# zicodasilva/cheetah_pose_estimation

Measured on AMD Instinct MI355X. Metric: frames/sec residual+Jacobian eval + full-traj solves/sec, 200-frame 6-cam seq, higher is better.
Workload: dtype f64; 1 GPU; cfg2: synthetic 200-frame x 6-cam x 25-marker sequences, phantom skeleton, const-accel model; frames=200, cams=6, markers=25, sequences_per_gpu=2048, parallelism=shard1 (independent sequences, no collective)

## Files before the change

cheetah_pose_estimation_amd/csrc/cpe_api.hip:

```cpp
#include <hip/hip_runtime.h>

#include <cmath>
#include <cstdio>
#include <cstdlib>
#include <cstring>
#include <functional>
#include <string>
#include <vector>
#include <algorithm>
#include <type_traits>

#include "cpe_kernels.hip"

static thread_local std::string g_err;
static cpe_status fail(cpe_status s, const std::string& m) { g_err = m; return s; }
#define HIPCHK(x)                                                                                         \
    do {                                                                                                  \
        hipError_t e_ = (x);                                                                              \
        if (e_ != hipSuccess) return fail(CPE_HIP_ERROR, std::string(#x) + ": " + hipGetErrorString(e_)); \
    } while (0)

struct cpe_handle {
    int device = 0;
    int n_cu = 256;
// ... 407 lines not shown
    return CPE_OK;
}

static void build_com_model(const cpe_skeleton* s, const cpe_camera* cams, int C, const cpe_options* o, std::vector<DevModel>& out, std::string& err) {
    if (!err.empty()) return;
    cpe_skeleton c = *s;
    c.n_markers = s->n_links;
    for (int i = 0; i < s->n_links && i < CPE_MAX_MARKERS; i++) {
        c.marker_link[i] = i;
        for (int d = 0; d < 3; d++) c.marker_off[i][d] = s->com[i][d];
    }
    const std::string keep = g_err;
    out.emplace_back();
    if (build_model(&c, cams, C, o, out.back(), false) != CPE_OK) { err = g_err; out.clear(); }
    g_err = keep;
}

template <bool RAGGED = false>
static auto frame_normal(bool plain) { return plain ? k_frame_normal<true, RAGGED> : k_frame_normal<false, RAGGED>; }
static size_t lds_fk(const DevModel& m) { return sizeof(double) * (m.nq + 6 * m.nl + 36 * m.nl + 3 * m.L + 23 * m.C); }
static size_t lds_normal(const DevModel& m, int gmm_k = 0, int gmm_dim = 0, bool shutter = false) {
    const bool plain = gmm_k == 0 && !shutter;
    size_t ov = CPE_MAX_SCOL * m.n_srow, hg = plain ? m.nu : m.nu * m.nu + m.nu;
    size_t camov = 6 * m.nl + 2 * m.nrev + 36 * m.n_trunk;
    if (camov < (size_t)22 * m.C) camov = (size_t)22 * m.C;
    size_t n = m.ns + camov + 3 * m.L + 3 * m.sv_n + GAM_STRIDE * m.nrev + (ov > hg ? ov : hg) +
               9 * m.L + 3 * m.mc_total;
    if (gmm_k > 0) n += CPE_NX + gmm_k * gmm_dim + CPE_MAX_GMM + CPE_NX;
    if (shutter) n += 15 * m.C + 6 * m.L + 6;
    return sizeof(double) * n;
}
template <bool RAGGED = false>
static auto frame_tracked(bool gmm) { return gmm ? k_frame_tracked<true, RAGGED> : k_frame_tracked<false, RAGGED>; }
static size_t lds_tracked(const DevModel& m, int gmm_k, int gmm_dim) {
    size_t n = m.ns + 6 * m.nl + 2 * m.nrev + 36 * m.n_trunk + GAM_STRIDE * m.nrev + m.nu + m.nu * m.nu + m.nu;
    if (gmm_k > 0) n += CPE_NX + gmm_k * gmm_dim + CPE_MAX_GMM + CPE_NX;
    return sizeof(double) * n;
}
template <class Fn>
static size_t lds_all(const cpe_handle* h, Fn&& lds) {
    size_t n = lds(h->hm);
    for (const DevModel& m : h->models) n = std::max(n, lds(m));
    return n;
}
static size_t lds_normal_all(const cpe_handle* h) { return lds_all(h, [h](const DevModel& m) { return lds_normal(m, h->gmm_k, h->gmm_dim); }); }
static size_t lds_fk(const cpe_handle* h, const RaggedArgs* rg) { return rg ? lds_all(h, [](const DevModel& m) { return lds_fk(m); }) : lds_fk(h->hm); }
static size_t lds_normal(const cpe_handle* h, const RaggedArgs* rg, bool shutter = false) {
    return rg ? lds_normal_all(h) : lds_normal(h->hm, h->gmm_k, h->gmm_dim, shutter);
}
static size_t lds_tracked(const cpe_handle* h, const RaggedArgs* rg) {
    return rg ? lds_all(h, [h](const DevModel& m) { return lds_tracked(m, h->gmm_k, h->gmm_dim); }) : lds_tracked(h->hm, h->gmm_k, h->gmm_dim);
}
static int n_models(const cpe_handle* h) { return h->models.empty() ? 1 : (int)h->models.size(); }
static int cams_max(const cpe_handle* h) {
    int c = h->hm.C;
    for (const DevModel& m : h->models) c = std::max(c, m.C);
    return c;
}

extern "C" {

const char* cpe_last_error(void) { return g_err.c_str(); }

void cpe_default_options(cpe_options* o) {
    o->h = 1.0 / 120.0; o->loss_a = 3.0; o->loss_b = 10.0; o->loss_c = 20.0; o->cost_scale = 1e-3;
    o->bound_penalty = 1e4; o->bound_tol = 1e-6; o->lambda0 = 1e-4; o->tol_step = 1e-8; o->tol_cost = 1e-9; o->max_iter = 200;
    o->curvature = 0; o->max_outer = 8; o->_pad = 0;
}

void cpe_destroy(cpe_handle* h);
static cpe_status create_impl(cpe_handle* h, const cpe_skeleton* skel, const cpe_camera* cams, int32_t n_cams, const cpe_options* opts,
                              const cpe_priors* priors, bool use_pri, const std::vector<DevModel>* models = nullptr) {
    const int device = h->device;
    if (models) { h->models = *models; h->hm = h->models[0]; }
    else {
        if (cpe_status s = build_model(skel, cams, n_cams, opts, h->hm); s != CPE_OK) return s;
        build_com_model(skel, cams, n_cams, opts, h->cmodels, h->com_err);
    }
    HIPCHK(hipSetDevice(device));
    {
        hipDeviceProp_t prop;
        HIPCHK(hipGetDeviceProperties(&prop, device));
        h->n_cu = prop.multiProcessorCount > 0 ? prop.multiProcessorCount : 256;
        const void* ks[] = {(const void*)&k_resjac<true, 4, 3, 2>, (const void*)&k_resjac<false, 4, 3, 2>,
                            (const void*)&k_resjac<true, 4, 4, 2>, (const void*)&k_resjac<false, 4, 4, 2>,
                            (const void*)&k_dyn_eval<>, (const void*)&k_dyn_assemble<>, (const void*)&k_dyn_schur<>, (const void*)&k_dyn_jac<>,
                            (const void*)&k_dyn_eval<true>, (const void*)&k_dyn_assemble<true>, (const void*)&k_dyn_schur<true>, (const void*)&k_dyn_jac<true>,
                            (const void*)&k_force_cov<>, (const void*)&k_force_cov<true>};
        for (const void* k : ks) {
            hipFuncAttributes fa;
            HIPCHK(hipFuncGetAttributes(&fa, k));
            HIPCHK(hipFuncSetAttribute(k, hipFuncAttributeMaxDynamicSharedMemorySize, 160 * 1024 - (int)fa.sharedSizeBytes));
        }
    }
    HIPCHK(hipStreamCreateWithFlags(&h->stream, hipStreamNonBlocking));
    HIPCHK(hipEventCreateWithFlags(&h->order_ev, hipEventDisableTiming));
    for (int i = 0; i < 2; i++) HIPCHK(hipEventCreateWithFlags(&h->poll_ev[i], hipEventDisableTiming));
    HIPCHK(hipHostMalloc(reinterpret_cast<void**>(&h->poll_host), 2 * sizeof(int), hipHostMallocDefault));
    HIPCHK(hipMalloc(&h->n_act, sizeof(int)));
    HIPCHK(hipMalloc(&h->dm, sizeof(DevModel) * n_models(h)));
    HIPCHK(hipMemcpy(h->dm, h->models.empty() ? &h->hm : h->models.data(), sizeof(DevModel) * n_models(h), hipMemcpyHostToDevice));
    HIPCHK(hipMalloc(&h->flag, sizeof(int)));
    if (!h->cmodels.empty()) {
        HIPCHK(hipMalloc(&h->dmc, sizeof(DevModel) * h->cmodels.size()));
        HIPCHK(hipMemcpy(h->dmc, h->cmodels.data(), sizeof(DevModel) * h->cmodels.size(), hipMemcpyHostToDevice));
    }
    if (use_pri) {
        if (h->hm.nu != CPE_NX) return fail(CPE_BAD_ARG, "learned priors need the 28 relative angles of the reference's skeleton");
        if (priors->gmm_k > 0 && priors->gmm_dim > h->hm.nu) return fail(CPE_BAD_ARG, "pose prior dimension exceeds the number of relative angles");
        std::vector<DevPriors> hp(1);
        DevPriors& P = hp[0];
        memset(&P, 0, sizeof(P));
        P.p = *priors;
        const int W = priors->lr_window, nu = CPE_NX;
        if (W > 0) {
            auto K = [&](int t, int p2, int j) -> double { return t == W ? (p2 == j ? 1.0 : 0.0) : -priors->lr_coef[p2][t * nu + j]; };
            for (int ta = 0; ta <= W; ta++)
                for (int tb = 0; tb <= ta; tb++)
                    for (int i = 0; i < nu; i++)
                        for (int j = 0; j < nu; j++) {
                            double a = 0.0;
                            for (int p2 = 0; p2 < nu; p2++) a += K(ta, p2, i) * priors->lr_w[p2] * K(tb, p2, j);
                            P.lr_PK[ta][tb][i * nu + j] = 2.0 * a;
                        }
            for (int k = 0; k <= W; k++)
                for (int ta = k; ta <= W; ta++)
                    for (int e = 0; e < nu * nu; e++) P.lr_HI[k][e] += P.lr_PK[ta][ta - k][e];
            for (int f = 0; f < W * nu; f++) {
                bool any = false;
                for (int p2 = 0; p2 < nu; p2++) { P.lr_coefT[f][p2] = priors->lr_coef[p2][f]; any = any || priors->lr_coef[p2][f] != 0.0; }
                if (any) P.lr_feat[P.lr_nf++] = (uint8_t)f;
            }
        }
        const DevModel& hm = h->hm;
        for (int i = 0; i < nu; i++)
            for (int side = 0; side < 2; side++) {
                const int kk = side == 0 ? i : hm.rel_ref_u[i];
                if (kk < 0) continue;
                const double sgn = side == 0 ? hm.rel_sign_u[i] : -hm.rel_sign_u[i];
                P.Xc[i][kk] += sgn;
                const int r = hm.rev_of_u[kk];
                if (r >= 0) P.Xc[i][hm.rev_body_u[r][1]] += sgn;
            }
        auto to_u = [&](const double* A, double* out) {
            std::vector<double> T((size_t)nu * nu);
            for (int r2 = 0; r2 < nu; r2++)
                for (int j = 0; j < nu; j++) { double a = 0.0; for (int c = 0; c < nu; c++) a += A[r2 * nu + c] * P.Xc[c][j]; T[(size_t)r2 * nu + j] = a; }
            for (int i = 0; i < nu; i++)
                for (int j = 0; j < nu; j++) { double a = 0.0; for (int r2 = 0; r2 < nu; r2++) a += P.Xc[r2][i] * T[(size_t)r2 * nu + j]; out[i * nu + j] = a; }
        };
        if (W > 0) {
            for (int ta = 0; ta <= W; ta++) for (int tb = 0; tb <= ta; tb++) to_u(P.lr_PK[ta][tb], P.lr_PKu[ta][tb]);
            for (int k = 0; k <= W; k++) to_u(P.lr_HI[k], P.lr_HIu[k]);
        }
        if (priors->gmm_k > 0) {
            const int D = priors->gmm_dim, off = nu - D;
            std::vector<double> A((size_t)nu * nu);
            for (int k = 0; k < priors->gmm_k; k++) {
                std::fill(A.begin(), A.end(), 0.0);
                for (int i = 0; i < D; i++)
                    for (int j = 0; j < D; j++) { A[(size_t)(off + i) * nu + off + j] = priors->gmm_P[k][i][j]; P.gmm_PT[k][j][i] = priors->gmm_P[k][i][j]; }
                to_u(A.data(), P.gmm_Q[k]);
            }
        }
        HIPCHK(hipMalloc(&h->pri, sizeof(DevPriors)));
        HIPCHK(hipMemcpy(h->pri, &P, sizeof(DevPriors), hipMemcpyHostToDevice));
        h->gmm_k = priors->gmm_k; h->gmm_dim = priors->gmm_dim; h->lr_window = W;
        h->pb = W > 3 ? W : 3;
// ... 122 lines not shown
cpe_status cpe_synchronize(cpe_handle* h) {
    if (!h) return fail(CPE_BAD_ARG, "null handle");
    HIPCHK(hipStreamSynchronize(h->stream));
    return CPE_OK;
}

cpe_status cpe_stream_wait(cpe_handle* h, void* other) {
    if (!h) return fail(CPE_BAD_ARG, "null handle");
    HIPCHK(hipSetDevice(h->device));
    HIPCHK(hipEventRecord(h->order_ev, (hipStream_t)other));
    HIPCHK(hipStreamWaitEvent(h->stream, h->order_ev, 0));
    return CPE_OK;
}
cpe_status cpe_stream_signal(cpe_handle* h, void* other) {
    if (!h) return fail(CPE_BAD_ARG, "null handle");
    HIPCHK(hipSetDevice(h->device));
    HIPCHK(hipEventRecord(h->order_ev, h->stream));
    HIPCHK(hipStreamWaitEvent((hipStream_t)other, h->order_ev, 0));
    return CPE_OK;
}

cpe_status cpe_profile_enable(cpe_handle* h, int32_t on) {
    if (!h) return fail(CPE_BAD_ARG, "null handle");
    h->prof = on != 0;
    for (int i = 0; i < CPE_PROFILE_SLOTS; i++) { h->prof_ms[i] = 0.0; h->prof_n[i] = 0; }
    return CPE_OK;
}
cpe_status cpe_profile_get(cpe_handle* h, double* ms, int64_t* launches) {
    if (!h || !ms || !launches) return fail(CPE_BAD_ARG, "null argument");
    for (int i = 0; i < CPE_PROFILE_SLOTS; i++) { ms[i] = h->prof_ms[i]; launches[i] = h->prof_n[i]; }
    return CPE_OK;
}
static void prof_begin(cpe_handle* h, int id) {
    if (!h->prof) return;
    hipEvent_t a = nullptr, b = nullptr;
    if (hipEventCreate(&a) != hipSuccess || hipEventCreate(&b) != hipSuccess) return;
    (void)hipEventRecord(a, h->stream);
    h->prof_spans.push_back({id, {a, b}});
}
static void prof_end(cpe_handle* h) {
    if (!h->prof || h->prof_spans.empty()) return;
    (void)hipEventRecord(h->prof_spans.back().second.second, h->stream);
}
static void prof_collect(cpe_handle* h) {
    for (auto& sp : h->prof_spans) {
        float ms = 0.f;
        if (hipEventElapsedTime(&ms, sp.second.first, sp.second.second) == hipSuccess) { h->prof_ms[sp.first] += ms; h->prof_n[sp.first]++; }
        (void)hipEventDestroy(sp.second.first); (void)hipEventDestroy(sp.second.second);
    }
    h->prof_spans.clear();
}

int32_t cpe_jacobian_slots(const cpe_handle* h) { return h ? h->hm.S : 0; }
cpe_status cpe_jacobian_layout(const cpe_handle* h, int32_t* slot_marker, int32_t* slot_dof) {
    if (!h || !slot_marker || !slot_dof) return fail(CPE_BAD_ARG, "null argument");
    for (int s = 0; s < h->hm.S; s++) { slot_marker[s] = h->hm.slot_marker[s]; slot_dof[s] = h->hm.slot_dof[s]; }
    return CPE_OK;
}
int32_t cpe_num_independent(const cpe_handle* h) { return h ? h->hm.nu : 0; }
cpe_status cpe_independent_dofs(const cpe_handle* h, int32_t* dofs) {
    if (!h || !dofs) return fail(CPE_BAD_ARG, "null argument");
    for (int k = 0; k < h->hm.nu; k++) dofs[k] = h->hm.indep[k];
    return CPE_OK;
}

static cpe_status frames(int32_t B, int32_t N, size_t* F) {
    if (B < 0 || N < 0) return fail(CPE_BAD_ARG, "negative size");
    *F = (size_t)B * N;
    if (*F > 0x7fffffffULL) return fail(CPE_BAD_ARG, "too many frames for one launch");
    return CPE_OK;
}

cpe_status cpe_eval_resjac(cpe_handle* h, int32_t B, int32_t N, const double* q, const double* meas, const double* weight,
                           double* r, double* J, double* eps, double* cost) {
    if (!h || !q || !meas || !r || !J || !eps) return fail(CPE_BAD_ARG, "null argument");
    if (cost && !weight) return fail(CPE_BAD_ARG, "cost requested without weights");
    size_t F;
    if (cpe_status s = frames(B, N, &F); s != CPE_OK) return s;
    if (F == 0) return CPE_OK;
    HIPCHK(hipSetDevice(h->device));
    const DevModel& m = h->hm;
    if (m.C * m.L > RJ_MAXPASS * WAVE) return fail(CPE_BAD_ARG, "cpe_eval_resjac supports at most 256 (camera, marker) pairs");
    constexpr int NW = 4;
    const size_t lds = sizeof(double) * (((rj_shared_doubles(m.C, m.L, m.S) + 1) & ~1) + (size_t)NW * rj_wave_doubles(m.C, m.L, m.nq, m.nl));
    int wg_per_cu = (int)((160 * 1024) / lds);
    if (wg_per_cu < 1) return fail(CPE_BAD_ARG, "model too large for the LDS of one workgroup");
    constexpr int variant = 2;
    if (wg_per_cu > variant) wg_per_cu = variant;
    long grid = (long)h->n_cu * wg_per_cu;
    const long need = (long)((F + NW - 1) / NW);
    if (grid > need) grid = need;
    const int npass = (m.C * m.L + WAVE - 1) / WAVE;
#define RJ_LAUNCH(COST, NP, OC) hipLaunchKernelGGL((k_resjac<COST, NW, NP, OC>), dim3((unsigned)grid), dim3(WAVE * NW), lds, h->stream, h->dm, N, (long)F, q, meas, weight, r, J, eps, cost)
    if (cost) { if (npass <= 3) RJ_LAUNCH(true, 3, 2); else RJ_LAUNCH(true, 4, 2); }
    else { if (npass <= 3) RJ_LAUNCH(false, 3, 2); else RJ_LAUNCH(false, 4, 2); }
#undef RJ_LAUNCH
    HIPCHK(hipGetLastError());
    return CPE_OK;
}

cpe_status cpe_project_joints(cpe_handle* h, int32_t B, int32_t N, double* q) {
    if (!h || !q) return fail(CPE_BAD_ARG, "null argument");
    size_t F;
    if (cpe_status s = frames(B, N, &F); s != CPE_OK) return s;
    if (F == 0) return CPE_OK;
    HIPCHK(hipSetDevice(h->device));
    HIPCHK(hipMemsetAsync(h->flag, 0, sizeof(int), h->stream));
    hipLaunchKernelGGL(k_project, dim3((unsigned)F), dim3(WAVE), sizeof(double) * (h->hm.nq + 6 * h->hm.nl), h->stream, h->dm, q, h->flag);
    HIPCHK(hipGetLastError());
    int fl = 0;
    HIPCHK(hipMemcpyAsync(&fl, h->flag, sizeof(int), hipMemcpyDeviceToHost, h->stream));
    HIPCHK(hipStreamSynchronize(h->stream));
    return fl ? CPE_NUMERICAL : CPE_OK;
}

cpe_status cpe_grf_fit(cpe_handle* h, const cpe_grf_options* opt, int32_t B, int32_t N, const double* q, const double* dq,
                       const double* ddq, const int32_t* contact, double* grfz, double* grfxy, double* residual) {
    if (!h || !opt || !q || !dq || !ddq || !contact || !grfz || !grfxy) return fail(CPE_BAD_ARG, "null argument");
    size_t F;
    if (cpe_status s = frames(B, N, &F); s != CPE_OK) return s;
    if (opt->n_feet < 1 || opt->n_feet > 4 || opt->iterations < 1 || !(opt->gravity > 0) || !(opt->force_max > 0) || !(opt->friction_ratio >= 0))
        return fail(CPE_BAD_ARG, "grf options out of range");
    for (int f = 0; f < opt->n_feet; f++)
        if (opt->foot_marker[f] < 0 || opt->foot_marker[f] >= h->hm.L) return fail(CPE_BAD_ARG, "foot marker index out of range");
    if (F == 0) return CPE_OK;
    HIPCHK(hipSetDevice(h->device));
    hipLaunchKernelGGL(k_grf, dim3((unsigned)((F + GRF_PACK - 1) / GRF_PACK)), dim3(WAVE), 0, h->stream, h->dm, *opt, F, q, dq, ddq, contact, grfz, grfxy, residual);
    HIPCHK(hipGetLastError());
    return CPE_OK;
}

cpe_status cpe_eom_rows(cpe_handle* h, const cpe_eom_options* opt, int32_t B, int32_t N, const double* q, const double* dq,
                        const double* ddq, double* rows) {
    if (!h || !opt || !q || !dq || !ddq || !rows) return fail(CPE_BAD_ARG, "null argument");
    size_t F;
    if (cpe_status s = frames(B, N, &F); s != CPE_OK) return s;
    if (F == 0) return CPE_OK;
    HIPCHK(hipSetDevice(h->device));
    if (!h->eom) HIPCHK(hipMalloc(&h->eom, sizeof(cpe_eom_options)));
    HIPCHK(hipMemcpyAsync(h->eom, opt, sizeof(cpe_eom_options), hipMemcpyHostToDevice, h->stream));
    hipLaunchKernelGGL(k_eom, dim3((unsigned)F), dim3(WAVE), 0, h->stream, h->dm, h->eom, F, q, dq, ddq, rows);
    HIPCHK(hipGetLastError());
    return CPE_OK;
}

cpe_status cpe_eom_residual(cpe_handle* h, const cpe_dyn_options* opt, int32_t B, int32_t N, const double* q, const double* dq,
                            const double* ddq, const double* tau, const double* lambda, const double* grf, double* residual) {
    if (!h || !opt || !q || !dq || !ddq || !residual) return fail(CPE_BAD_ARG, "null argument");
    if (opt->n_feet < 0 || opt->n_feet > 4 || opt->n_motors < 0 || opt->n_motors > 32) return fail(CPE_BAD_ARG, "dynamics options out of range");
    for (int f = 0; f < opt->n_feet; f++) if (opt->foot_marker[f] < 0 || opt->foot_marker[f] >= h->hm.L) return fail(CPE_BAD_ARG, "foot marker index out of range");
    for (int m = 0; m < opt->n_motors; m++)
        if (opt->motor_first[m] < 0 || opt->motor_first[m] >= h->hm.nl || opt->motor_second[m] < 0 || opt->motor_second[m] >= h->hm.nl ||
            opt->motor_axis[m] < 0 || opt->motor_axis[m] > 2) return fail(CPE_BAD_ARG, "motor definition out of range");
    size_t F;
    if (cpe_status s = frames(B, N, &F); s != CPE_OK) return s;
    cpe_status s = cpe_eom_rows(h, &opt->eom, B, N, q, dq, ddq, residual);
    if (s != CPE_OK) return s;
    if (F == 0 || (!tau && !lambda && !grf)) return CPE_OK;
    if (!h->dyn) HIPCHK(hipMalloc(&h->dyn, sizeof(cpe_dyn_options)));
    HIPCHK(hipMemcpyAsync(h->dyn, opt, sizeof(cpe_dyn_options), hipMemcpyHostToDevice, h->stream));
    int n_con = 0;
    for (int j = 0; j < h->hm.nj; j++) n_con += h->hm.joint_kind[j] == CPE_JOINT_REVOLUTE_Y ? 2 : 1;
    hipLaunchKernelGGL(k_dyn_forces, dim3((unsigned)F), dim3(WAVE), 0, h->stream, h->dm, h->dyn, F, q, tau, lambda, grf, n_con, residual);
    HIPCHK(hipGetLastError());
    return CPE_OK;
}

cpe_status cpe_forward_kinematics(cpe_handle* h, int32_t B, int32_t N, const double* q, double* positions, double* com) {
    if (!h || !q || !positions) return fail(CPE_BAD_ARG, "null argument");
    size_t F;
    if (cpe_status s = frames(B, N, &F); s != CPE_OK) return s;
    if (F == 0) return CPE_OK;
    HIPCHK(hipSetDevice(h->device));
    hipLaunchKernelGGL(k_fk, dim3((unsigned)F), dim3(WAVE), lds_fk(h->hm), h->stream, h->dm, q, positions, com);
    HIPCHK(hipGetLastError());
    return CPE_OK;
}

cpe_status cpe_marker_velocities(cpe_handle* h, int32_t B, int32_t N, const double* q, const double* dq, double* velocities) {
// ... 1784 lines not shown
```

cheetah_pose_estimation_amd/csrc/cpe_kernels.hip:

```cpp
#include <hip/hip_runtime.h>

#include "cpe_device.h"


__device__ __forceinline__ void wave_sincos(const DevModel* __restrict__ M, const double* sq, double* ssc, int lane) {
    if (lane < 3 * M->nl) {
        double s, c;
        sincos(sq[3 + lane], &s, &c);
        ssc[2 * lane] = s; ssc[2 * lane + 1] = c;
    }
}

__device__ __forceinline__ void wave_rotations(const DevModel* __restrict__ M, const double* ssc, double* sR, int lane) {
    for (int t = lane; t < 4 * M->nl; t += WAVE) rot_kind(ssc + 6 * (t >> 2), t & 3, sR + 9 * t);
}

__device__ __forceinline__ void wave_markers(const DevModel* __restrict__ M, const double* sq, const double* sR,
                                             double* spos, int lane) {
    if (lane < M->L) {
        double p0 = sq[0], p1 = sq[1], p2 = sq[2];
        const int n = M->chain_len[lane];
        for (int k = 0; k < n; k++) {
            const double* R = sR + 36 * M->chain_link[lane][k];
            const double v0 = M->chain_vec[lane][k][0], v1 = M->chain_vec[lane][k][1], v2 = M->chain_vec[lane][k][2];
// ... 74 lines not shown
__device__ __forceinline__ void wave_tail_roll(double* sq, double* ssc, int hj_n, int fwx, int lane) {
    for (int level = 0; level < 2; level++) {
        if (lane < hj_n && ((fwx >> 16) & 1) == level) {
            const int p = fwx & 255, c = (fwx >> 8) & 255;
            double a[3], phi, sphi, cphi;
            rot_ycol(ssc + 6 * p, a);
            hooke_roll(a, ssc[6 * c + 2], ssc[6 * c + 3], ssc[6 * c + 4], ssc[6 * c + 5], phi, sphi, cphi);
            sq[3 + 3 * c] = phi;
            ssc[6 * c] = sphi; ssc[6 * c + 1] = cphi;
        }
        wave_lds_sync();
    }
}

__device__ __forceinline__ void wave_trunk_rotations(const DevModel* __restrict__ M, const double* ssc, double* sR, int fwy, int lane) {
    if (lane < 4 * M->n_trunk) rot_kind(ssc + 6 * fwy, lane & 3, sR + 9 * lane);
    for (int t = WAVE + lane; t < 4 * M->n_trunk; t += WAVE) rot_kind(ssc + 6 * M->trunk_link[t >> 2], t & 3, sR + 9 * t);
}

__device__ __forceinline__ void wave_leg_vectors(const double* ssa, double* sdyn, int svn, int fww, const double (&svv)[3][3], int lane) {
    if (lane < svn) {
        double d0 = 0.0, d1 = 0.0, d2 = 0.0;
        if ((fww & 3) == 0) {
            const int cnt = (fww >> 2) & 3;
#pragma unroll
            for (int i = 0; i < 3; i++) {
                const int r = (fww >> (4 + 6 * i)) & 63;
                const double sa = ssa[2 * r], ca = ssa[2 * r + 1];
                if (i < cnt) { d0 += ca * svv[i][0] + sa * svv[i][2]; d1 += svv[i][1]; d2 += -sa * svv[i][0] + ca * svv[i][2]; }
            }
        } else {
            const int r = (fww >> 4) & 63;
            const double sa = ssa[2 * r], ca = ssa[2 * r + 1];
            d0 = -sa * svv[0][0] + ca * svv[0][2]; d2 = -ca * svv[0][0] - sa * svv[0][2];
        }
        sdyn[3 * lane] = d0; sdyn[3 * lane + 1] = d1; sdyn[3 * lane + 2] = d2;
    }
}

__device__ __forceinline__ void wave_hooke_srows(const double* sR, double* sSv, int hk_n, int2 hkw, int lane) {
    for (int level = 0; level < 2; level++) {
        if (lane < hk_n && ((hkw.x >> 16) & 1) == level) {
            const double* Rp = sR + 36 * (hkw.x & 63); const double* Rc = sR + 36 * ((hkw.x >> 6) & 63);
            const double y0 = Rp[1], y1 = Rp[4], y2 = Rp[7];
            const double z0 = Rc[2], z1 = Rc[5], z2 = Rc[8];
            const double* Dcphi = Rc + 9;
            const double gphi = y0 * Dcphi[2] + y1 * Dcphi[5] + y2 * Dcphi[8];
            const int kind = (hkw.x >> 12) & 3, ang = (hkw.x >> 14) & 3;
            double direct = 0.0;
            if (kind == 0) { const double* D = Rc + 9 * (1 + ang); direct = y0 * D[2] + y1 * D[5] + y2 * D[8]; }
            else if (kind == 1) { const double* D = Rp + 9 * (1 + ang); direct = D[1] * z0 + D[4] * z1 + D[7] * z2; }
            double val = -direct / gphi;
            const int ch = (hkw.y & 0xFFFF) - 1;
            if (ch >= 0) {
                const double* Dpphi = Rp + 9;
                const double t0 = -(Dpphi[1] * z0 + Dpphi[4] * z1 + Dpphi[7] * z2) / gphi;
                val += t0 * sSv[ch];
            }
            sSv[hkw.y >> 16] = val;
        }
        wave_lds_sync();
    }
}

#define RJ_MAXPASS 4

#define RJ_GLOBAL __attribute__((address_space(1)))
typedef double rj_v2d __attribute__((ext_vector_type(2)));
template <typename T>
__device__ __forceinline__ RJ_GLOBAL T* rj_sbase(T* p) {
    RJ_GLOBAL T* g = (RJ_GLOBAL T*)p;
    asm("" : "+s"(g));
    return g;
}

__host__ __device__ inline int rj_shared_doubles(int C, int L, int S) {
    return 23 * C + 10 + 3 * S + (2 * S + 1) / 2 + 3 * L * CPE_MAX_CHAIN + (L * CPE_MAX_CHAIN + 1) / 2 + (L + 1) / 2;
}
__host__ __device__ inline int rj_wave_doubles(int C, int L, int nq, int nl) {
    const int a = 6 * C * L, b = nq + 6 * nl + 36 * nl;
    return ((a > b ? a : b) + 3 * L + 3) & ~1;
}

template <bool WANT_COST, int NW, int NPASS, int OCC>
__global__ __launch_bounds__(WAVE * NW, (OCC * NW) / 4) void k_resjac(const DevModel* __restrict__ M, int N, long F,
                                                      const double* __restrict__ q, const double* __restrict__ meas,
                                                      const double* __restrict__ weight, double* __restrict__ r,
                                                      double* __restrict__ J, double* __restrict__ eps,
                                                      double* __restrict__ cost) {
    extern __shared__ double smem[];
    const int tid = threadIdx.x, lane = tid & 63;
    const int wave = __builtin_amdgcn_readfirstlane(tid >> 6);
    const int nq = M->nq, nl = M->nl, L = M->L, C = M->C, S = M->S, CL = C * L;
    double* scam = smem;
    double* sident = scam + 23 * C;
    double* slv = sident + 10;
    int* sli = reinterpret_cast<int*>(slv + 3 * S);
    double* chv = slv + 3 * S + (2 * S + 1) / 2;
    int* chr = reinterpret_cast<int*>(chv + 3 * L * CPE_MAX_CHAIN);
    int* sclen = reinterpret_cast<int*>(chv + 3 * L * CPE_MAX_CHAIN + (L * CPE_MAX_CHAIN + 1) / 2);
    double* wbase = smem + ((rj_shared_doubles(C, L, S) + 1) & ~1);
    const int nA = rj_wave_doubles(C, L, nq, nl) - ((3 * L + 3) & ~1) + 0;
    double* wv = wbase + wave * rj_wave_doubles(C, L, nq, nl);
    double* sq = wv;
    double* ssc = sq + nq;
    double* sR = ssc + 6 * nl;
    double* sG = wv;
    double* spos = wv + nA;

    for (int t = tid; t < 23 * C; t += WAVE * NW) scam[t] = reinterpret_cast<const double*>(M->cam)[t];
    if (tid < 9) sident[tid] = (tid == 0 || tid == 4 || tid == 8) ? 1.0 : 0.0;
    for (int s = tid; s < S; s += WAVE * NW) {
        const int l = M->slot_marker[s], cpos = M->slot_cpos[s];
        sli[S + s] = l;
        if (cpos < 0) {
            const int ax = cpos == -2 ? 3 : M->slot_dof[s];
            slv[s] = ax == 0 ? 1.0 : 0.0; slv[S + s] = ax == 1 ? 1.0 : 0.0; slv[2 * S + s] = ax == 2 ? 1.0 : 0.0; sli[s] = -1;
        } else {
            slv[s] = M->chain_vec[l][cpos][0]; slv[S + s] = M->chain_vec[l][cpos][1]; slv[2 * S + s] = M->chain_vec[l][cpos][2];
            sli[s] = 9 * (4 * M->chain_link[l][cpos] + 1 + M->slot_ang[s]);
        }
    }
    for (int t = tid; t < L * CPE_MAX_CHAIN; t += WAVE * NW) {
        const int k = t / L, l = t - k * L;
        const bool on = k < M->chain_len[l];
        chv[t] = on ? M->chain_vec[l][k][0] : 0.0;
        chv[L * CPE_MAX_CHAIN + t] = on ? M->chain_vec[l][k][1] : 0.0;
        chv[2 * L * CPE_MAX_CHAIN + t] = on ? M->chain_vec[l][k][2] : 0.0;
        chr[t] = on ? 36 * M->chain_link[l][k] : 0;
    }
    for (int t = tid; t < L; t += WAVE * NW) sclen[t] = M->chain_len[t];
    const double ih2 = M->ih2, la = M->loss_a, lb = M->loss_b, lc = M->loss_c;
    __syncthreads();

    const cpe_camera* cams = reinterpret_cast<const cpe_camera*>(scam);
    int pcam[NPASS], ppos[NPASS], gofs[5];
#pragma unroll
    for (int p = 0; p < NPASS; p++) {
        const int t = lane + WAVE * p;
        const int c = t < CL ? t / L : 0;
        pcam[p] = c; ppos[p] = t < CL ? 3 * (t - c * L) : 0;
    }
#pragma unroll
    for (int i = 0; i < 5; i++) {
        const int s = lane + WAVE * i;
        gofs[i] = s < S ? 6 * sli[S + s] : 0;
    }
    const unsigned Fu = (unsigned)F, wstride = gridDim.x * NW;
    unsigned f = blockIdx.x * NW + wave;

    const rj_v2d* meas2 = reinterpret_cast<const rj_v2d*>(meas);
    unsigned n = (unsigned)(f % N);
    const unsigned dn = (unsigned)(wstride % N);
    const unsigned ulane = lane;
    double qreg = 0.0;
    if (f < Fu && lane < nq) qreg = rj_sbase(q + (unsigned long)f * (unsigned)nq)[ulane];
    __builtin_amdgcn_s_waitcnt(0x0F70);

    while (f < Fu) {
        __builtin_amdgcn_s_setprio(2);
        if (lane < nq) sq[lane] = qreg;
        const unsigned fn = f + wstride;
        const unsigned long fq = (unsigned long)f * (unsigned)nq, fcl = (unsigned long)f * (unsigned)CL, fj = (unsigned long)f * (unsigned)(C * S);
        const bool has_prev = n >= 3u;
        double qn = 0.0, qp1 = 0.0, qp2 = 0.0, qp3 = 0.0;
        rj_v2d mz[NPASS];
        double wz[NPASS];
        if (lane < nq) {
            if (fn < Fu) qn = rj_sbase(q + (unsigned long)fn * (unsigned)nq)[ulane];
            if (has_prev) { qp1 = rj_sbase(q + (fq - nq))[ulane]; qp2 = rj_sbase(q + (fq - 2 * nq))[ulane]; qp3 = rj_sbase(q + (fq - 3 * nq))[ulane]; }
        }
        RJ_GLOBAL const rj_v2d* measf = rj_sbase(meas2 + fcl);
        RJ_GLOBAL const double* weightf = WANT_COST ? rj_sbase(weight + fcl) : nullptr;
#pragma unroll
        for (int p = 0; p < NPASS; p++) {
            const int t = lane + WAVE * p;
            mz[p] = rj_v2d{0.0, 0.0}; wz[p] = 0.0;
            if (t < CL) { mz[p] = measf[ulane + WAVE * p]; if (WANT_COST) wz[p] = weightf[ulane + WAVE * p]; }
        }
        wave_lds_sync();
        if (lane < 3 * nl) {
            double sn, cs;
            sincos(sq[3 + lane], &sn, &cs);
            ssc[2 * lane] = sn; ssc[2 * lane + 1] = cs;
        }
        wave_lds_sync();
        for (int t = lane; t < 4 * nl; t += WAVE) rot_kind(ssc + 6 * (t >> 2), t & 3, sR + 9 * t);
        wave_lds_sync();
        {
            const int half = lane >= L ? 1 : 0, l = lane - half * L;
            double p0 = 0.0, p1 = 0.0, p2 = 0.0;
            if (lane < 2 * L) {
                if (!half) { p0 = sq[0]; p1 = sq[1]; p2 = sq[2]; }
                const int n = sclen[l];
                const int KL = L * CPE_MAX_CHAIN;
                for (int k = half; k < n; k += 2) {
                    const int t = k * L + l;
                    const double v0 = chv[t], v1 = chv[KL + t], v2 = chv[2 * KL + t];
                    const double* R = sR + chr[t];
                    p0 += R[0] * v0 + R[1] * v1 + R[2] * v2;
                    p1 += R[3] * v0 + R[4] * v1 + R[5] * v2;
                    p2 += R[6] * v0 + R[7] * v1 + R[8] * v2;
                }
            }
            const int partner = (lane + L) & (WAVE - 1);
            const double o0 = __shfl(p0, partner, WAVE), o1 = __shfl(p1, partner, WAVE), o2 = __shfl(p2, partner, WAVE);
            if (lane < L) { spos[3 * lane] = p0 + o0; spos[3 * lane + 1] = p1 + o1; spos[3 * lane + 2] = p2 + o2; }
        }
        double dp0[5], dp1[5], dp2[5];
#pragma unroll
        for (int i = 0; i < 5; i++) {
            const int s = lane + WAVE * i;
            dp0[i] = dp1[i] = dp2[i] = 0.0;
            if (s < S) {
                const int doff = sli[s];
                const double v0 = slv[s], v1 = slv[S + s], v2 = slv[2 * S + s];
                const double* D = doff < 0 ? sident : sR + doff;
                dp0[i] = D[0] * v0 + D[1] * v1 + D[2] * v2;
                dp1[i] = D[3] * v0 + D[4] * v1 + D[5] * v2;
                dp2[i] = D[6] * v0 + D[7] * v1 + D[8] * v2;
            }
        }
        wave_lds_sync();

        RJ_GLOBAL rj_v2d* rf = rj_sbase(reinterpret_cast<rj_v2d*>(r) + fcl);
        double fc = 0.0;
        double2 uv[NPASS];
#pragma unroll
        for (int p = 0; p < NPASS; p++) {
            __builtin_amdgcn_sched_barrier(0);
            const int t = lane + WAVE * p;
            uv[p] = make_double2(0.0, 0.0);
            if (t < CL) {
                const double* pl = spos + ppos[p];
                double u, v, G[6];
                project_point(cams[pcam[p]], pl[0], pl[1], pl[2], u, v, G);
                uv[p] = make_double2(u, v);
                double2* Gd = reinterpret_cast<double2*>(sG + 6 * t);
                Gd[0] = make_double2(G[0], G[1]); Gd[1] = make_double2(G[2], G[3]); Gd[2] = make_double2(G[4], G[5]);
            }
        }
        wave_lds_sync();
        __builtin_amdgcn_s_setprio(0);
        __builtin_amdgcn_s_waitcnt(0x0F70);
        asm volatile("" : "+v"(qp1), "+v"(qp2), "+v"(qp3), "+v"(qn));
#pragma unroll
        for (int p = 0; p < NPASS; p++) {
            const int t = lane + WAVE * p;
            if (t < CL) {
                const double e0 = uv[p].x - mz[p].x, e1 = uv[p].y - mz[p].y;
                rf[ulane + WAVE * p] = rj_v2d{e0, e1};
                if (WANT_COST) {
                    const double w = cams[pcam[p]].mult * wz[p];
                    fc += robust_loss(w * e0, la, lb, lc, 0, false).rho + robust_loss(w * e1, la, lb, lc, 0, false).rho;
                }
            }
        }
        const int nfull = S >> 6;
        for (int c = 0; c < C; c++) {
            const double* Gc = sG + 6 * c * L;
            RJ_GLOBAL rj_v2d* Jc = rj_sbase(reinterpret_cast<rj_v2d*>(J) + (fj + (unsigned)(c * S)));
            double2 g0[5], g1[5], g2[5];
#pragma unroll
            for (int i = 0; i < 5; i++) {
                const double2* G = reinterpret_cast<const double2*>(Gc + gofs[i]);
                g0[i] = G[0]; g1[i] = G[1]; g2[i] = G[2];
            }
            rj_v2d val[5];
#pragma unroll
            for (int i = 0; i < 5; i++) {
                val[i].x = g0[i].x * dp0[i] + g0[i].y * dp1[i] + g1[i].x * dp2[i];
                val[i].y = g1[i].y * dp0[i] + g2[i].x * dp1[i] + g2[i].y * dp2[i];
                asm volatile("" : "+v"(val[i]));
            }
#pragma unroll
            for (int i = 0; i < 5; i++) {
                if (i < nfull || lane + WAVE * i < S) {
#ifdef CPE_RJ_NOSTORE
                    if (val[i].x == 1.2345e300) Jc[ulane + WAVE * i] = val[i];
#else
                    __builtin_nontemporal_store(val[i], &Jc[ulane + WAVE * i]);
#endif
                }
            }
        }
        if (WANT_COST) {
            fc = wave_sum(fc);
            if (lane == 0) cost[f] = fc;
        }
        if (lane < nq) {
            double e = 0.0;
            if (has_prev) e = (qreg - 3.0 * qp1 + 3.0 * qp2 - qp3) * ih2;
            rj_sbase(eps + fq)[ulane] = e;
        }
        qreg = qn;
        f = fn;
        n += dn;
        if (n >= (unsigned)N) n -= (unsigned)N;
        wave_lds_sync();
    }
}

__global__ __launch_bounds__(WAVE) void k_fk(const DevModel* __restrict__ M, const double* __restrict__ q,
                                             double* __restrict__ positions, double* __restrict__ com) {
    extern __shared__ double smem[];
    const int lane = threadIdx.x;
    const int nq = M->nq, nl = M->nl, L = M->L;
    double* sq = smem;
    double* ssc = sq + nq;
    double* sR = ssc + 6 * nl;
    double* spos = sR + 36 * nl;
    const size_t f = blockIdx.x;
    if (lane < nq) sq[lane] = q[f * nq + lane];
    wave_lds_sync();
    wave_sincos(M, sq, ssc, lane);
    wave_lds_sync();
    for (int t = lane; t < nl; t += WAVE) rot_kind(ssc + 6 * t, 0, sR + 36 * t);
    wave_lds_sync();
    wave_markers(M, sq, sR, spos, lane);
    wave_lds_sync();
    for (int t = lane; t < 3 * L; t += WAVE) positions[f * (size_t)(3 * L) + t] = spos[t];
    if (com) {
        double c0 = 0.0, c1 = 0.0, c2 = 0.0;
        if (lane < nl) {
            const double* R = sR + 36 * lane;
            double p0 = R[0] * M->com[lane][0] + R[1] * M->com[lane][1] + R[2] * M->com[lane][2];
            double p1 = R[3] * M->com[lane][0] + R[4] * M->com[lane][1] + R[5] * M->com[lane][2];
            double p2 = R[6] * M->com[lane][0] + R[7] * M->com[lane][1] + R[8] * M->com[lane][2];
            int k = lane;
            while (M->parent[k] >= 0) {
                const int p = M->parent[k];
                const double* Rp = sR + 36 * p;
                p0 += Rp[0] * M->attach[k][0] + Rp[1] * M->attach[k][1] + Rp[2] * M->attach[k][2];
                p1 += Rp[3] * M->attach[k][0] + Rp[4] * M->attach[k][1] + Rp[5] * M->attach[k][2];
                p2 += Rp[6] * M->attach[k][0] + Rp[7] * M->attach[k][1] + Rp[8] * M->attach[k][2];
                k = p;
            }
            const double m = M->mass[lane];
            c0 = m * (p0 + sq[0]); c1 = m * (p1 + sq[1]); c2 = m * (p2 + sq[2]);
        }
        c0 = wave_sum(c0); c1 = wave_sum(c1); c2 = wave_sum(c2);
        if (lane == 0) {
            com[3 * f] = c0 * M->inv_total_mass; com[3 * f + 1] = c1 * M->inv_total_mass; com[3 * f + 2] = c2 * M->inv_total_mass;
        }
    }
}

__global__ __launch_bounds__(WAVE) void k_marker_vel(const DevModel* __restrict__ M, const double* __restrict__ q,
                                                     const double* __restrict__ dq, double* __restrict__ vel) {
    extern __shared__ double smem[];
    const int lane = threadIdx.x;
    const int nq = M->nq, nl = M->nl, L = M->L;
    double* sq = smem;
    double* sdq = sq + nq;
    double* ssc = sdq + nq;
    double* sR = ssc + 6 * nl;
    const size_t f = blockIdx.x;
    if (lane < nq) { sq[lane] = q[f * nq + lane]; sdq[lane] = dq[f * nq + lane]; }
    wave_lds_sync();
    wave_sincos(M, sq, ssc, lane);
    wave_lds_sync();
    wave_rotations(M, ssc, sR, lane);
    wave_lds_sync();
    if (lane < L) {
        double v0 = 0.0, v1 = 0.0, v2 = 0.0;
        for (int s = M->slot_off[lane]; s < M->slot_off[lane + 1]; s++) {
            double d0, d1, d2;
            slot_dp(M, sR, s, d0, d1, d2);
            const double w = sdq[M->slot_dof[s]];
            v0 += d0 * w; v1 += d1 * w; v2 += d2 * w;
        }
        double* o = vel + (f * (size_t)L + lane) * 3;
        o[0] = v0; o[1] = v1; o[2] = v2;
    }
}

__global__ __launch_bounds__(WAVE) void k_reproject(const DevModel* __restrict__ M, const double* __restrict__ positions,
                                                    double* __restrict__ uv) {
    const int L = M->L, CL = M->C * L;
    const size_t f = blockIdx.x;
    const double* P = positions + f * (size_t)(3 * L);
// ... 132 lines not shown
```

Before: 151.4 million frames/s.

## Add contiguous per-wave frame runs to resjac kernel with lookahead successor indexing

Lets each workgroup process a run of K consecutive frame groups before striding over the grid, selected by a template flag and a host heuristic or environment variable. The default run length stays at one. Frame and sequence-position successors are now computed one iteration ahead, using a host-precomputed modular jump instead of a per-iteration modulo. This is meant to improve locality of the previous-frame q reads and to take scalar index math off the critical path. In exchange it doubles the kernel instantiations and adds some control-flow complexity.

```diff
diff --git a/cheetah_pose_estimation_amd/csrc/cpe_api.hip b/cheetah_pose_estimation_amd/csrc/cpe_api.hip
--- a/cheetah_pose_estimation_amd/csrc/cpe_api.hip
+++ b/cheetah_pose_estimation_amd/csrc/cpe_api.hip
@@ -513,8 +513,10 @@
         hipDeviceProp_t prop;
         HIPCHK(hipGetDeviceProperties(&prop, device));
         h->n_cu = prop.multiProcessorCount > 0 ? prop.multiProcessorCount : 256;
-        const void* ks[] = {(const void*)&k_resjac<true, 4, 3, 2>, (const void*)&k_resjac<false, 4, 3, 2>,
-                            (const void*)&k_resjac<true, 4, 4, 2>, (const void*)&k_resjac<false, 4, 4, 2>,
+        const void* ks[] = {(const void*)&k_resjac<true, 4, 3, 2, false>, (const void*)&k_resjac<false, 4, 3, 2, false>,
+                            (const void*)&k_resjac<true, 4, 4, 2, false>, (const void*)&k_resjac<false, 4, 4, 2, false>,
+                            (const void*)&k_resjac<true, 4, 3, 2, true>, (const void*)&k_resjac<false, 4, 3, 2, true>,
+                            (const void*)&k_resjac<true, 4, 4, 2, true>, (const void*)&k_resjac<false, 4, 4, 2, true>,
                             (const void*)&k_dyn_eval<>, (const void*)&k_dyn_assemble<>, (const void*)&k_dyn_schur<>, (const void*)&k_dyn_jac<>,
                             (const void*)&k_dyn_eval<true>, (const void*)&k_dyn_assemble<true>, (const void*)&k_dyn_schur<true>, (const void*)&k_dyn_jac<true>,
                             (const void*)&k_force_cov<>, (const void*)&k_force_cov<true>};
@@ -803,6 +805,7 @@
     const DevModel& m = h->hm;
     if (m.C * m.L > RJ_MAXPASS * WAVE) return fail(CPE_BAD_ARG, "cpe_eval_resjac supports at most 256 (camera, marker) pairs");
     constexpr int NW = 4;
+    constexpr long RJ_RUN_DEFAULT = 1;
     const size_t lds = sizeof(double) * (((rj_shared_doubles(m.C, m.L, m.S) + 1) & ~1) + (size_t)NW * rj_wave_doubles(m.C, m.L, m.nq, m.nl));
     int wg_per_cu = (int)((160 * 1024) / lds);
     if (wg_per_cu < 1) return fail(CPE_BAD_ARG, "model too large for the LDS of one workgroup");
@@ -811,11 +814,21 @@
     long grid = (long)h->n_cu * wg_per_cu;
     const long need = (long)((F + NW - 1) / NW);
     if (grid > need) grid = need;
+    auto busiest = [&](long K) { const long runs = (need + K - 1) / K; return (runs + grid - 1) / grid * K; };
+    long K = RJ_RUN_DEFAULT;
+    if (const char* e = getenv("CPE_RJ_RUN")) K = std::max(1L, strtol(e, nullptr, 10));
+    else while (K > 1 && 100 * busiest(K) > 103 * busiest(1)) K--;
+    if (K > need) K = need;
+    const long runs = (need + K - 1) / K;
+    if (grid > runs) grid = runs;
+    const long njump = (grid * NW * K - NW * (K - 1)) % N;
     const int npass = (m.C * m.L + WAVE - 1) / WAVE;
-#define RJ_LAUNCH(COST, NP, OC) hipLaunchKernelGGL((k_resjac<COST, NW, NP, OC>), dim3((unsigned)grid), dim3(WAVE * NW), lds, h->stream, h->dm, N, (long)F, q, meas, weight, r, J, eps, cost)
+#define RJ_LAUNCH_K(COST, NP, OC, RUNS) hipLaunchKernelGGL((k_resjac<COST, NW, NP, OC, RUNS>), dim3((unsigned)grid), dim3(WAVE * NW), lds, h->stream, h->dm, N, (long)F, (int)K, (int)njump, q, meas, weight, r, J, eps, cost)
+#define RJ_LAUNCH(COST, NP, OC) do { if (K > 1) RJ_LAUNCH_K(COST, NP, OC, true); else RJ_LAUNCH_K(COST, NP, OC, false); } while (0)
     if (cost) { if (npass <= 3) RJ_LAUNCH(true, 3, 2); else RJ_LAUNCH(true, 4, 2); }
     else { if (npass <= 3) RJ_LAUNCH(false, 3, 2); else RJ_LAUNCH(false, 4, 2); }
 #undef RJ_LAUNCH
+#undef RJ_LAUNCH_K
     HIPCHK(hipGetLastError());
     return CPE_OK;
 }
diff --git a/cheetah_pose_estimation_amd/csrc/cpe_kernels.hip b/cheetah_pose_estimation_amd/csrc/cpe_kernels.hip
--- a/cheetah_pose_estimation_amd/csrc/cpe_kernels.hip
+++ b/cheetah_pose_estimation_amd/csrc/cpe_kernels.hip
@@ -180,8 +180,8 @@
     return ((a > b ? a : b) + 3 * L + 3) & ~1;
 }
 
-template <bool WANT_COST, int NW, int NPASS, int OCC>
-__global__ __launch_bounds__(WAVE * NW, (OCC * NW) / 4) void k_resjac(const DevModel* __restrict__ M, int N, long F,
+template <bool WANT_COST, int NW, int NPASS, int OCC, bool RUNS>
+__global__ __launch_bounds__(WAVE * NW, (OCC * NW) / 4) void k_resjac(const DevModel* __restrict__ M, int N, long F, int runlen, int njump,
                                                       const double* __restrict__ q, const double* __restrict__ meas,
                                                       const double* __restrict__ weight, double* __restrict__ r,
                                                       double* __restrict__ J, double* __restrict__ eps,
@@ -244,12 +244,36 @@
         const int s = lane + WAVE * i;
         gofs[i] = s < S ? 6 * sli[S + s] : 0;
     }
-    const unsigned Fu = (unsigned)F, wstride = gridDim.x * NW;
-    unsigned f = blockIdx.x * NW + wave;
+    const unsigned Fu = (unsigned)F, R = (unsigned)runlen * NW;
+    const unsigned nruns = (Fu - 1u) / R + 1u;
+    unsigned grid = gridDim.x;
+    asm("" : "+s"(grid));
+    unsigned run = blockIdx.x, jrun = 0;
+    unsigned f = run * R + wave;
 
     const rj_v2d* meas2 = reinterpret_cast<const rj_v2d*>(meas);
-    unsigned n = (unsigned)(f % N);
-    const unsigned dn = (unsigned)(wstride % N);
+    unsigned n = f % (unsigned)N;
+    const unsigned dn = (unsigned)NW % (unsigned)N;
+    const unsigned fjump = grid * R - (unsigned)NW * ((unsigned)runlen - 1u);
+    auto succ = [&](unsigned x, unsigned xn, unsigned& y, unsigned& yn) {
+        if constexpr (!RUNS) {
+            y = x + fjump;
+            yn = xn + (unsigned)njump;
+            if (yn >= (unsigned)N) yn -= (unsigned)N;
+            return;
+        }
+        const bool last = ++jrun == (unsigned)runlen;
+        y = x + (last ? fjump : (unsigned)NW);
+        yn = xn + (last ? (unsigned)njump : dn);
+        if (yn >= (unsigned)N) yn -= (unsigned)N;
+        if (last) {
+            jrun = 0;
+            run += grid;
+            if (run >= nruns) y = ~0u;
+        }
+    };
+    unsigned fn, nn;
+    succ(f, n, fn, nn);
     const unsigned ulane = lane;
     double qreg = 0.0;
     if (f < Fu && lane < nq) qreg = rj_sbase(q + (unsigned long)f * (unsigned)nq)[ulane];
@@ -258,7 +282,6 @@
     while (f < Fu) {
         __builtin_amdgcn_s_setprio(2);
         if (lane < nq) sq[lane] = qreg;
-        const unsigned fn = f + wstride;
         const unsigned long fq = (unsigned long)f * (unsigned)nq, fcl = (unsigned long)f * (unsigned)CL, fj = (unsigned long)f * (unsigned)(C * S);
         const bool has_prev = n >= 3u;
         double qn = 0.0, qp1 = 0.0, qp2 = 0.0, qp3 = 0.0;
@@ -340,6 +363,12 @@
         }
         wave_lds_sync();
         __builtin_amdgcn_s_setprio(0);
+        unsigned fnn, nnn;
+        if constexpr (RUNS) asm volatile("" : "+s"(run));
+        else asm volatile("" : "+s"(fn));
+        succ(fn, nn, fnn, nnn);
+        asm volatile("" : "+s"(fnn));
+        asm volatile("" : "+s"(nnn));
         __builtin_amdgcn_s_waitcnt(0x0F70);
         asm volatile("" : "+v"(qp1), "+v"(qp2), "+v"(qp3), "+v"(qn));
 #pragma unroll
@@ -392,9 +421,8 @@
             rj_sbase(eps + fq)[ulane] = e;
         }
         qreg = qn;
-        f = fn;
-        n += dn;
-        if (n >= (unsigned)N) n -= (unsigned)N;
+        f = fn; n = nn;
+        fn = fnn; nn = nnn;
         wave_lds_sync();
     }
 }
```

Result: no change. 151.7 million frames/s, median of 6 (+0.2%).
